# TheShadow29/VidSitu

Measured on AMD Instinct MI355X. Metric: clips/s (10s@32x224x224) SlowFast+TxEnc fwd+bwd, higher is better.
Workload: dtype bf16

## Files before the change

### vidsitu_amd/csrc/conv_stem.hip

```cpp
#include "common.h"

#define ST_TH 8
#define ST_TW 16
#define ST_PH 21
#define ST_PW 40
#define ST_ROWB (ST_PW * 8)
#define ST_FRAMEB (ST_PH * ST_ROWB)
#define ST_TC 4

struct StemP {
  const uint16_t* x;
  const uint16_t* w;
  uint16_t* y;
  const float* scale;
  const float* shift;
  float* stats;
  int N, T, H, W, Ho, Wo, Cout, kT, y_ld, flags;
  int tilesH, tilesW, tchunks, ntiles;
};

template <int NT>
__global__ __launch_bounds__(256) void stem_conv_kernel(StemP p) {
  extern __shared__ __attribute__((aligned(16))) char smem[];
  constexpr int CP = NT * 16;
  const int K = p.kT * 7 * 32;
  const int wpitch = K * 2 + 16;
  char* wlds = smem;
  char* patch = smem + ((CP * wpitch + 15) & ~15);
  const int patch_bytes = p.kT * ST_FRAMEB;
  float* E = (float*)(patch + ((patch_bytes + 15) & ~15));
  float* statbuf = E + 128 * CP;

  const int tid = threadIdx.x;
  {
    const int chunks_per_row = K / 8;
    for (int i = tid; i < CP * chunks_per_row; i += 256) {
      const int r = i / chunks_per_row, c = i - r * chunks_per_row;
      *(u32x4*)(wlds + r * wpitch + c * 16) = *(const u32x4*)(p.w + (long long)r * K + c * 8);
    }
  }
  const int wave = tid >> 6, lane = tid & 63;
  const int lr = lane & 15, lq = lane >> 4;
  const int pT = p.kT >> 1;

  auto stage_frame = [&](int n, int ti, int hi0, int wi0) __attribute__((always_inline)) {
    const int slot = ((ti % p.kT) + p.kT) % p.kT;
    char* dst = patch + slot * ST_FRAMEB;
    const bool tin = (unsigned)ti < (unsigned)p.T;
    const uint16_t* src = p.x + (((long long)n * p.T + (tin ? ti : 0)) * p.H) * (long long)p.W * 4;
    uint2 v[4];
#pragma unroll
    for (int u = 0; u < 4; ++u) {
      const int i = tid + u * 256;
      const int r = i / ST_PW, c = i - r * ST_PW;
      const int hi = hi0 + r, wi = wi0 + c;
      v[u] = make_uint2(0u, 0u);
      if (i < ST_PH * ST_PW && tin && (unsigned)hi < (unsigned)p.H && (unsigned)wi < (unsigned)p.W)
        v[u] = *(const uint2*)(src + ((long long)hi * p.W + wi) * 4);
    }
#pragma unroll
    for (int u = 0; u < 4; ++u) {
      const int i = tid + u * 256;
      if (i < ST_PH * ST_PW) *(uint2*)(dst + i * 8) = v[u];
    }
  };

  for (int item = blockIdx.x; item < p.ntiles; item += gridDim.x) {
    int t = item;
    const int tc = t % p.tchunks;
    t /= p.tchunks;
    const int tw = t % p.tilesW;
    t /= p.tilesW;
    const int th = t % p.tilesH;
    const int n = t / p.tilesH;
    const int ho0 = th * ST_TH, wo0 = tw * ST_TW;
    const int hi0 = 2 * ho0 - 3, wi0 = 2 * wo0 - 3;
    const int to_beg = tc * ST_TC, to_end = min(p.T, to_beg + ST_TC);
   for (int to = to_beg; to < to_end; ++to) {
    const int tile = ((n * p.T + to) * p.tilesH + th) * p.tilesW + tw;
    __syncthreads();
    if (to == to_beg) {
      for (int dt = 0; dt < p.kT; ++dt) stage_frame(n, to - pT + dt, hi0, wi0);
    } else {
      stage_frame(n, to + pT, hi0, wi0);
    }
    __syncthreads();

    f32x4 acc[2][NT];
#pragma unroll
    for (int a = 0; a < 2; ++a)
#pragma unroll
      for (int b = 0; b < NT; ++b) acc[a][b] = (f32x4){0.f, 0.f, 0.f, 0.f};

    int slot = (to - pT) % p.kT;
    if (slot < 0) slot += p.kT;
    int ks = 0;
    for (int dt = 0; dt < p.kT; ++dt) {
      const char* fbase = patch + slot * ST_FRAMEB + (2 * lr + 2 * lq) * 8;
      for (int dh = 0; dh < 7; ++dh, ++ks) {
        bf16x8 af[2], bfr[NT];
#pragma unroll
        for (int a = 0; a < 2; ++a) {
          const int hol = wave * 2 + a;
          af[a] = *(const bf16x8*)(fbase + (2 * hol + dh) * ST_ROWB);
        }
#pragma unroll
        for (int b = 0; b < NT; ++b)
          bfr[b] = *(const bf16x8*)(wlds + (b * 16 + lr) * wpitch + (ks * 32 + lq * 8) * 2);
#pragma unroll
        for (int a = 0; a < 2; ++a)
#pragma unroll
          for (int b = 0; b < NT; ++b)
            acc[a][b] = __builtin_amdgcn_mfma_f32_16x16x32_bf16(af[a], bfr[b], acc[a][b], 0, 0, 0);
      }
      if (++slot == p.kT) slot = 0;
    }

#pragma unroll
    for (int a = 0; a < 2; ++a) {
      const int ho = ho0 + wave * 2 + a;
#pragma unroll
      for (int r = 0; r < 4; ++r) {
        const int wo = wo0 + lq * 4 + r;
        if (ho >= p.Ho || wo >= p.Wo) {
#pragma unroll
          for (int b = 0; b < NT; ++b) acc[a][b][r] = 0.f;
        }
      }
    }
    if (p.flags & VS_CONV_STATS) {
#pragma unroll
      for (int b = 0; b < NT; ++b) {
        float s = 0.f, q = 0.f;
#pragma unroll
        for (int a = 0; a < 2; ++a)
#pragma unroll
          for (int r = 0; r < 4; ++r) {
            const float v = acc[a][b][r];
            s += v;
            q += v * v;
          }
        s += __shfl_xor(s, 16, 64);
        q += __shfl_xor(q, 16, 64);
        s += __shfl_xor(s, 32, 64);
        q += __shfl_xor(q, 32, 64);
        if (lq == 0) {
          statbuf[wave * CP + b * 16 + lr] = s;
          statbuf[4 * CP + wave * CP + b * 16 + lr] = q;
        }
      }
    }
#pragma unroll
    for (int b = 0; b < NT; ++b) {
      const int col = b * 16 + lr;
      float sc = 1.f, sh = 0.f;
      if ((p.flags & VS_CONV_AFFINE) && col < p.Cout) {
        sc = p.scale[col];
        sh = p.shift[col];
      }
#pragma unroll
      for (int a = 0; a < 2; ++a)
#pragma unroll
        for (int r = 0; r < 4; ++r) {
          const int row = (wave * 2 + a) * 16 + lq * 4 + r;
          E[row * CP + col] = acc[a][b][r] * sc + sh;
        }
    }
    __syncthreads();
    if ((p.flags & VS_CONV_STATS) && tid < p.Cout) {
      float s = 0.f, q = 0.f;
#pragma unroll
      for (int w = 0; w < 4; ++w) {
        s += statbuf[w * CP + tid];
        q += statbuf[4 * CP + w * CP + tid];
      }
      float* dst = p.stats + (long long)tile * 2 * p.Cout;
      dst[tid] = s;
      dst[p.Cout + tid] = q;
    }
    const int cpr = p.Cout >> 3;
    for (int idx = tid; idx < 128 * cpr; idx += 256) {
      const int row = idx / cpr, c8 = idx - row * cpr;
      const int ho = ho0 + (row >> 4), wo = wo0 + (row & 15);
      if (ho < p.Ho && wo < p.Wo) {
        float v[8];
        const float4 v0 = *(const float4*)(E + row * CP + c8 * 8);
        const float4 v1 = *(const float4*)(E + row * CP + c8 * 8 + 4);
        v[0] = v0.x; v[1] = v0.y; v[2] = v0.z; v[3] = v0.w;
        v[4] = v1.x; v[5] = v1.y; v[6] = v1.z; v[7] = v1.w;
        if (p.flags & VS_CONV_RELU) {
#pragma unroll
          for (int e = 0; e < 8; ++e) v[e] = fmaxf(v[e], 0.f);
        }
        const long long pos = (((long long)n * p.T + to) * p.Ho + ho) * p.Wo + wo;
        *(uint4*)(p.y + pos * p.y_ld + c8 * 8) = pack8_bf16(v);
      }
    }
   }
  }
}

#define SP_TH 16
#define SP_PH 37
#define SP_FRAMEB (SP_PH * ST_ROWB)
#define SP_TC 8

__global__ __launch_bounds__(512) void stem_pair_kernel(StemP p) {
  extern __shared__ __attribute__((aligned(16))) char smem[];
  const int kT = p.kT, KT1 = kT + 1, pT = kT >> 1;
  const int K = kT * 7 * 32, K2 = KT1 * 7 * 32;
  const int wpitch = K2 * 2 + 16;
  char* wlds = smem;
  char* patch = smem + ((16 * wpitch + 15) & ~15);
  float* E = (float*)(patch + ((KT1 * SP_FRAMEB + 15) & ~15));
  float* statbuf = E + 256 * 16;
  const int tid = threadIdx.x;
  {
    const int cpr = K2 / 8;
    for (int i = tid; i < 16 * cpr; i += 512) {
      const int r = i / cpr, c = i - r * cpr;
      const int ks = c >> 2, sub = c & 3;
      const int dtp = ks / 7, dh = ks - dtp * 7;
      const int j = r >> 3, co = r & 7, dt = dtp - j;
      u32x4 v = {0u, 0u, 0u, 0u};
      if (dt >= 0 && dt < kT && co < p.Cout)
        v = *(const u32x4*)(p.w + (long long)co * K + ((dt * 7 + dh) * 32 + sub * 8));
      *(u32x4*)(wlds + r * wpitch + c * 16) = v;
    }
  }
  const int wave = tid >> 6, lane = tid & 63;
  const int lr = lane & 15, lq = lane >> 4;
  const int tilesH16 = (p.Ho + SP_TH - 1) / SP_TH;

  auto slot_of = [&](int ti) { return ((ti % KT1) + KT1) % KT1; };
  auto frame_load = [&](int n, int ti, int hi0, int wi0, uint2* v) __attribute__((always_inline)) {
    const bool tin = (unsigned)ti < (unsigned)p.T;
    const uint16_t* src = p.x + (((long long)n * p.T + (tin ? ti : 0)) * p.H) * (long long)p.W * 4;
#pragma unroll
    for (int u = 0; u < 3; ++u) {
      const int i = tid + u * 512;
      const int r = i / ST_PW, c = i - r * ST_PW;
      const int hi = hi0 + r, wi = wi0 + c;
      v[u] = make_uint2(0u, 0u);
      if (i < SP_PH * ST_PW && tin && (unsigned)hi < (unsigned)p.H && (unsigned)wi < (unsigned)p.W)
        v[u] = *(const uint2*)(src + ((long long)hi * p.W + wi) * 4);
    }
  };
  auto frame_store = [&](int ti, const uint2* v) __attribute__((always_inline)) {
    char* dst = patch + slot_of(ti) * SP_FRAMEB;
#pragma unroll
    for (int u = 0; u < 3; ++u) {
      const int i = tid + u * 512;
      if (i < SP_PH * ST_PW) *(uint2*)(dst + i * 8) = v[u];
    }
  };

  for (int item = blockIdx.x; item < p.ntiles; item += gridDim.x) {
    int t = item;
    const int tc = t % p.tchunks;
    t /= p.tchunks;
    const int tw = t % p.tilesW;
    t /= p.tilesW;
    const int th = t % tilesH16;
    const int n = t / tilesH16;
    const int ho0 = th * SP_TH, wo0 = tw * ST_TW;
    const int hi0 = 2 * ho0 - 3, wi0 = 2 * wo0 - 3;
    const int to_beg = tc * SP_TC, to_end = min(p.T, to_beg + SP_TC);
    __syncthreads();
    for (int f = 0; f < KT1; ++f) {
      uint2 v[3];
      frame_load(n, to_beg - pT + f, hi0, wi0, v);
      frame_store(to_beg - pT + f, v);
    }
    __syncthreads();
    for (int to0 = to_beg; to0 < to_end; to0 += 2) {
      const bool more = to0 + 2 < to_end;
      uint2 nf0[3], nf1[3];
      if (more) {
        frame_load(n, to0 - pT + KT1, hi0, wi0, nf0);
        frame_load(n, to0 - pT + KT1 + 1, hi0, wi0, nf1);
      }
      f32x4 acc[2];
      acc[0] = (f32x4){0.f, 0.f, 0.f, 0.f};
      acc[1] = (f32x4){0.f, 0.f, 0.f, 0.f};
      int slot = slot_of(to0 - pT);
      const char* wrow = wlds + lr * wpitch + lq * 16;
      for (int dtp = 0; dtp < KT1; ++dtp) {
        const char* fbase = patch + slot * SP_FRAMEB + (2 * lr + 2 * lq) * 8 + (4 * wave) * ST_ROWB;
        bf16x8 af[9];
#pragma unroll
        for (int r = 0; r < 9; ++r) af[r] = *(const bf16x8*)(fbase + r * ST_ROWB);
#pragma unroll
        for (int dh = 0; dh < 7; ++dh) {
          const bf16x8 bfr = *(const bf16x8*)(wrow + (dtp * 7 + dh) * 64);
          acc[0] = __builtin_amdgcn_mfma_f32_16x16x32_bf16(af[dh], bfr, acc[0], 0, 0, 0);
          acc[1] = __builtin_amdgcn_mfma_f32_16x16x32_bf16(af[dh + 2], bfr, acc[1], 0, 0, 0);
        }
        if (++slot == KT1) slot = 0;
      }
      const int j = lr >> 3, co = lr & 7;
      const bool fok = to0 + j < p.T && co < p.Cout;
#pragma unroll
      for (int a = 0; a < 2; ++a) {
        const int ho = ho0 + wave * 2 + a;
#pragma unroll
        for (int r = 0; r < 4; ++r) {
          const int wo = wo0 + lq * 4 + r;
          if (ho >= p.Ho || wo >= p.Wo || !fok) acc[a][r] = 0.f;
        }
      }
      if (p.flags & VS_CONV_STATS) {
        float s = 0.f, q = 0.f;
#pragma unroll
        for (int a = 0; a < 2; ++a)
#pragma unroll
          for (int r = 0; r < 4; ++r) {
            const float v = acc[a][r];
            s += v;
            q += v * v;
          }
        s += __shfl_xor(s, 16, 64);
        q += __shfl_xor(q, 16, 64);
        s += __shfl_xor(s, 32, 64);
        q += __shfl_xor(q, 32, 64);
        if (lq == 0) {
          statbuf[wave * 16 + lr] = s;
          statbuf[8 * 16 + wave * 16 + lr] = q;
        }
      }
      {
        float sc = 1.f, sh = 0.f;
        if ((p.flags & VS_CONV_AFFINE) && co < p.Cout) {
          sc = p.scale[co];
          sh = p.shift[co];
        }
#pragma unroll
        for (int a = 0; a < 2; ++a)
#pragma unroll
          for (int r = 0; r < 4; ++r) E[((wave * 2 + a) * 16 + lq * 4 + r) * 16 + lr] = acc[a][r] * sc + sh;
      }
      __syncthreads();
      if ((p.flags & VS_CONV_STATS) && tid < 32) {
        const int h = tid >> 4, col = tid & 15, jj = col >> 3, cc = col & 7;
        const int th8 = 2 * th + h;
        if (cc < p.Cout && to0 + jj < p.T && th8 < p.tilesH) {
          float s = 0.f, q = 0.f;
#pragma unroll
          for (int w = 0; w < 4; ++w) {
            s += statbuf[(4 * h + w) * 16 + col];
            q += statbuf[8 * 16 + (4 * h + w) * 16 + col];
          }
          const int tile = ((n * p.T + to0 + jj) * p.tilesH + th8) * p.tilesW + tw;
          float* dst = p.stats + (long long)tile * 2 * p.Cout;
          dst[cc] = s;
          dst[p.Cout + cc] = q;
        }
      }
      {
        const int row = tid >> 1, jj = tid & 1;
        const int ho = ho0 + (row >> 4), wo = wo0 + (row & 15);
        if (ho < p.Ho && wo < p.Wo && to0 + jj < p.T) {
          float v[8];
          const float4 v0 = *(const float4*)(E + row * 16 + jj * 8);
          const float4 v1 = *(const float4*)(E + row * 16 + jj * 8 + 4);
          v[0] = v0.x; v[1] = v0.y; v[2] = v0.z; v[3] = v0.w;
          v[4] = v1.x; v[5] = v1.y; v[6] = v1.z; v[7] = v1.w;
          if (p.flags & VS_CONV_RELU) {
#pragma unroll
            for (int e = 0; e < 8; ++e) v[e] = fmaxf(v[e], 0.f);
          }
          const long long pos = (((long long)n * p.T + to0 + jj) * p.Ho + ho) * p.Wo + wo;
          *(uint4*)(p.y + pos * p.y_ld) = pack8_bf16(v);
        }
      }
      __syncthreads();
      if (more) {
        frame_store(to0 - pT + KT1, nf0);
        frame_store(to0 - pT + KT1 + 1, nf1);
      }
      __syncthreads();
    }
  }
}

template <int KT>
__global__ __launch_bounds__(256) void stem_pair_reg_kernel(StemP p) {
  extern __shared__ __attribute__((aligned(16))) char smem[];
  constexpr int KT1 = KT + 1, pT = KT >> 1, NKS = KT1 * 7;
  constexpr int K = KT * 7 * 32;
  char* patch = smem;
  float* E = (float*)(patch + ((KT1 * ST_FRAMEB + 15) & ~15));
  float* statbuf = E + 128 * 16;
  const int tid = threadIdx.x;
  const int wave = tid >> 6, lane = tid & 63;
  const int lr = lane & 15, lq = lane >> 4;
  const int j = lr >> 3, co = lr & 7;

  bf16x8 bfr[NKS];
#pragma unroll
  for (int ks = 0; ks < NKS; ++ks) {
    const int dtp = ks / 7, dh = ks - dtp * 7;
    const int dt = dtp - j;
    u32x4 v = {0u, 0u, 0u, 0u};
    if (dt >= 0 && dt < KT && co < p.Cout)
      v = *(const u32x4*)(p.w + (long long)co * K + ((dt * 7 + dh) * 32 + lq * 8));
    bfr[ks] = __builtin_bit_cast(bf16x8, v);
  }

  auto slot_of = [](int ti) { return ((ti % KT1) + KT1) % KT1; };
  auto frame_load = [&](int n, int ti, int hi0, int wi0, uint2* v) __attribute__((always_inline)) {
    const bool tin = (unsigned)ti < (unsigned)p.T;
    const uint16_t* src = p.x + (((long long)n * p.T + (tin ? ti : 0)) * p.H) * (long long)p.W * 4;
#pragma unroll
    for (int u = 0; u < 4; ++u) {
      const int i = tid + u * 256;
      const int r = i / ST_PW, c = i - r * ST_PW;
      const int hi = hi0 + r, wi = wi0 + c;
      v[u] = make_uint2(0u, 0u);
      if (i < ST_PH * ST_PW && tin && (unsigned)hi < (unsigned)p.H && (unsigned)wi < (unsigned)p.W)
        v[u] = *(const uint2*)(src + ((long long)hi * p.W + wi) * 4);
    }
  };
  auto frame_store = [&](int ti, const uint2* v) __attribute__((always_inline)) {
    char* dst = patch + slot_of(ti) * ST_FRAMEB;
#pragma unroll
    for (int u = 0; u < 4; ++u) {
      const int i = tid + u * 256;
      if (i < ST_PH * ST_PW) *(uint2*)(dst + i * 8) = v[u];
    }
  };

  for (int item = blockIdx.x; item < p.ntiles; item += gridDim.x) {
    int t = item;
    const int tc = t % p.tchunks;
    t /= p.tchunks;
    const int tw = t % p.tilesW;
    t /= p.tilesW;
    const int th = t % p.tilesH;
    const int n = t / p.tilesH;
    const int ho0 = th * ST_TH, wo0 = tw * ST_TW;
    const int hi0 = 2 * ho0 - 3, wi0 = 2 * wo0 - 3;
    const int to_beg = tc * SP_TC, to_end = min(p.T, to_beg + SP_TC);
    __syncthreads();
    for (int f = 0; f < KT1; ++f) {
      uint2 v[4];
      frame_load(n, to_beg - pT + f, hi0, wi0, v);
      frame_store(to_beg - pT + f, v);
    }
    __syncthreads();
    for (int to0 = to_beg; to0 < to_end; to0 += 2) {
      const bool more = to0 + 2 < to_end;
      uint2 nf0[4], nf1[4];
      if (more) {
        frame_load(n, to0 - pT + KT1, hi0, wi0, nf0);
        frame_load(n, to0 - pT + KT1 + 1, hi0, wi0, nf1);
      }
      f32x4 acc[2];
      acc[0] = (f32x4){0.f, 0.f, 0.f, 0.f};
      acc[1] = (f32x4){0.f, 0.f, 0.f, 0.f};
      int slot = slot_of(to0 - pT);
#pragma unroll
      for (int dtp = 0; dtp < KT1; ++dtp) {
        const char* fbase = patch + slot * ST_FRAMEB + (2 * lr + 2 * lq) * 8 + (4 * wave) * ST_ROWB;
        bf16x8 af[9];
#pragma unroll
        for (int r = 0; r < 9; ++r) af[r] = *(const bf16x8*)(fbase + r * ST_ROWB);
#pragma unroll
        for (int dh = 0; dh < 7; ++dh) {
          acc[0] = __builtin_amdgcn_mfma_f32_16x16x32_bf16(af[dh], bfr[dtp * 7 + dh], acc[0], 0, 0, 0);
          acc[1] = __builtin_amdgcn_mfma_f32_16x16x32_bf16(af[dh + 2], bfr[dtp * 7 + dh], acc[1], 0, 0, 0);
        }
        if (++slot == KT1) slot = 0;
      }
      const bool fok = to0 + j < p.T && co < p.Cout;
#pragma unroll
      for (int a = 0; a < 2; ++a) {
        const int ho = ho0 + wave * 2 + a;
#pragma unroll
        for (int r = 0; r < 4; ++r) {
          const int wo = wo0 + lq * 4 + r;
          if (ho >= p.Ho || wo >= p.Wo || !fok) acc[a][r] = 0.f;
        }
      }
      if (p.flags & VS_CONV_STATS) {
        float s = 0.f, q = 0.f;
#pragma unroll
        for (int a = 0; a < 2; ++a)
#pragma unroll
          for (int r = 0; r < 4; ++r) {
            const float v = acc[a][r];
            s += v;
            q += v * v;
          }
        s += __shfl_xor(s, 16, 64);
        q += __shfl_xor(q, 16, 64);
        s += __shfl_xor(s, 32, 64);
        q += __shfl_xor(q, 32, 64);
        if (lq == 0) {
          statbuf[wave * 16 + lr] = s;
          statbuf[4 * 16 + wave * 16 + lr] = q;
        }
      }
      {
        float sc = 1.f, sh = 0.f;
        if ((p.flags & VS_CONV_AFFINE) && co < p.Cout) {
          sc = p.scale[co];
          sh = p.shift[co];
        }
#pragma unroll
        for (int a = 0; a < 2; ++a)
#pragma unroll
          for (int r = 0; r < 4; ++r) E[((wave * 2 + a) * 16 + lq * 4 + r) * 16 + lr] = acc[a][r] * sc + sh;
      }
      __syncthreads();
      if ((p.flags & VS_CONV_STATS) && tid < 16) {
        const int jj = tid >> 3, cc = tid & 7;
        if (cc < p.Cout && to0 + jj < p.T) {
          float s = 0.f, q = 0.f;
#pragma unroll
          for (int w = 0; w < 4; ++w) {
            s += statbuf[w * 16 + tid];
            q += statbuf[4 * 16 + w * 16 + tid];
          }
          const int tile = ((n * p.T + to0 + jj) * p.tilesH + th) * p.tilesW + tw;
          float* dst = p.stats + (long long)tile * 2 * p.Cout;
          dst[cc] = s;
          dst[p.Cout + cc] = q;
        }
      }
      {
        const int row = tid >> 1, jj = tid & 1;
        const int ho = ho0 + (row >> 4), wo = wo0 + (row & 15);
        if (ho < p.Ho && wo < p.Wo && to0 + jj < p.T) {
          float v[8];
          const float4 v0 = *(const float4*)(E + row * 16 + jj * 8);
          const float4 v1 = *(const float4*)(E + row * 16 + jj * 8 + 4);
          v[0] = v0.x; v[1] = v0.y; v[2] = v0.z; v[3] = v0.w;
          v[4] = v1.x; v[5] = v1.y; v[6] = v1.z; v[7] = v1.w;
          if (p.flags & VS_CONV_RELU) {
#pragma unroll
            for (int e = 0; e < 8; ++e) v[e] = fmaxf(v[e], 0.f);
          }
          const long long pos = (((long long)n * p.T + to0 + jj) * p.Ho + ho) * p.Wo + wo;
          *(uint4*)(p.y + pos * p.y_ld) = pack8_bf16(v);
        }
      }
      __syncthreads();
      if (more) {
        frame_store(to0 - pT + KT1, nf0);
        frame_store(to0 - pT + KT1 + 1, nf1);
      }
      __syncthreads();
    }
  }
}

static size_t stem_pair_smem(int kT) {
  const int K2 = (kT + 1) * 7 * 32;
  const size_t w = ((size_t)16 * (K2 * 2 + 16) + 15) & ~(size_t)15;
  const size_t patch = ((size_t)(kT + 1) * SP_FRAMEB + 15) & ~(size_t)15;
  return w + patch + (size_t)256 * 16 * 4 + (size_t)2 * 8 * 16 * 4;
}

static size_t stem_smem(int CP, int kT) {
  const int K = kT * 7 * 32;
  const size_t w = ((size_t)CP * (K * 2 + 16) + 15) & ~(size_t)15;
  const size_t patch = ((size_t)kT * ST_FRAMEB + 15) & ~(size_t)15;
  return w + patch + (size_t)128 * CP * 4 + (size_t)2 * 4 * CP * 4;
}

extern "C" int vs_stem_stats_rows(int N, int T, int H, int W) {
  const int Ho = (H + 6 - 7) / 2 + 1, Wo = (W + 6 - 7) / 2 + 1;
  return N * T * ((Ho + ST_TH - 1) / ST_TH) * ((Wo + ST_TW - 1) / ST_TW);
}

extern "C" int vs_stem_conv_fwd(const void* x4, const void* wp, void* y, int N, int T, int H, int W,
                                int Cout, int kT, int y_ld, int flags, const float* scale,
                                const float* shift, float* stats_partial, void* stream) {
  VS_CHECK_ARG(x4 && wp && y, "null tensor");
  VS_CHECK_ARG(Cout % 8 == 0 && Cout <= 64 && y_ld % 8 == 0 && y_ld >= Cout, "Cout in {8..64}, pitch % 8");
  VS_CHECK_ARG(kT == 1 || kT == 3 || kT == 5, "kT in {1,3,5}");
  VS_CHECK_ARG(!(flags & VS_CONV_AFFINE) || (scale && shift), "AFFINE needs scale/shift");
  VS_CHECK_ARG(!(flags & VS_CONV_STATS) || stats_partial, "STATS needs stats_partial");
  VS_CHECK_ARG(!(flags & VS_CONV_RESIDUAL), "no residual on a stem");
  StemP p;
  p.x = (const uint16_t*)x4;
  p.w = (const uint16_t*)wp;
  p.y = (uint16_t*)y;
  p.scale = scale;
  p.shift = shift;
  p.stats = stats_partial;
  p.N = N; p.T = T; p.H = H; p.W = W;
  p.Ho = (H + 6 - 7) / 2 + 1;
  p.Wo = (W + 6 - 7) / 2 + 1;
  p.Cout = Cout; p.kT = kT; p.y_ld = y_ld; p.flags = flags;
  p.tilesH = (p.Ho + ST_TH - 1) / ST_TH;
  p.tilesW = (p.Wo + ST_TW - 1) / ST_TW;
  p.tchunks = (T + ST_TC - 1) / ST_TC;
  p.ntiles = N * p.tilesH * p.tilesW * p.tchunks;
  const int CP = (Cout + 15) / 16 * 16;
  hipStream_t st = (hipStream_t)stream;
  static const int pair_on = [] { const char* e = getenv("VS_STEM_PAIR"); return e ? atoi(e) : 1; }();
  if (pair_on == 1 && Cout == 8 && kT >= 3 && T >= 2) {
    p.tchunks = (T + SP_TC - 1) / SP_TC;
    p.ntiles = N * p.tilesH * p.tilesW * p.tchunks;
    const int grid2 = p.ntiles < 512 ? p.ntiles : 512;
    const size_t smem2 = (((size_t)(kT + 1) * ST_FRAMEB + 15) & ~(size_t)15) + (size_t)128 * 16 * 4 + 2 * 4 * 16 * 4;
    if (kT == 5) hipLaunchKernelGGL(stem_pair_reg_kernel<5>, dim3(grid2), dim3(256), smem2, st, p);
    else hipLaunchKernelGGL(stem_pair_reg_kernel<3>, dim3(grid2), dim3(256), smem2, st, p);
    VS_CHECK_LAUNCH();
    return VS_OK;
  }
  if (pair_on && Cout == 8 && kT >= 3 && T >= 2) {
    static bool attr_done = false;
    if (!attr_done) {
      (void)hipFuncSetAttribute((const void*)stem_pair_kernel, hipFuncAttributeMaxDynamicSharedMemorySize, 160 * 1024);
      attr_done = true;
    }
    p.tchunks = (T + SP_TC - 1) / SP_TC;
    p.ntiles = N * ((p.Ho + SP_TH - 1) / SP_TH) * p.tilesW * p.tchunks;
    const int grid2 = p.ntiles < 256 ? p.ntiles : 256;
    hipLaunchKernelGGL(stem_pair_kernel, dim3(grid2), dim3(512), stem_pair_smem(kT), st, p);
    VS_CHECK_LAUNCH();
    return VS_OK;
  }
  const size_t smem = stem_smem(CP, kT);
  int grid = p.ntiles < 512 ? p.ntiles : 512;
#define LAUNCH_STEM(NT_)                                                                         \
  do {                                                                                           \
    static bool attr_done = false;                                                               \
    if (!attr_done) {                                                                            \
      (void)hipFuncSetAttribute((const void*)stem_conv_kernel<NT_>,                              \
                                hipFuncAttributeMaxDynamicSharedMemorySize, 160 * 1024);         \
      attr_done = true;                                                                          \
    }                                                                                            \
    hipLaunchKernelGGL((stem_conv_kernel<NT_>), dim3(grid), dim3(256), smem, st, p);             \
  } while (0)
  switch (CP / 16) {
    case 1: LAUNCH_STEM(1); break;
    case 2: LAUNCH_STEM(2); break;
    case 3: LAUNCH_STEM(3); break;
    default: LAUNCH_STEM(4); break;
  }
#undef LAUNCH_STEM
  VS_CHECK_LAUNCH();
  return VS_OK;
}

typedef __attribute__((ext_vector_type(4))) short st_s16x4;
typedef __attribute__((address_space(3))) st_s16x4 st_lds_s16x4;
typedef __attribute__((ext_vector_type(8))) short st_s16x8;

__device__ __forceinline__ bf16x8 st_tr_pair(const char* p0, const char* p1) {
  const st_s16x4 lo = __builtin_amdgcn_ds_read_tr16_b64_v4i16((st_lds_s16x4*)p0);
  const st_s16x4 hi = __builtin_amdgcn_ds_read_tr16_b64_v4i16((st_lds_s16x4*)p1);
  const st_s16x8 v = __builtin_shufflevector(lo, hi, 0, 1, 2, 3, 4, 5, 6, 7);
  return __builtin_bit_cast(bf16x8, v);
}

struct StemWgP {
  const uint16_t* x;
  const uint16_t* dy;
  float* slabs;
  int N, T, H, W, Ho, Wo, Cout, kT, dy_ld;
  int tilesH, tilesW, tchunks, nitems;
};

template <int MT, int NTW>
__global__ __launch_bounds__(256) void stem_wgrad_kernel(StemWgP p) {
  extern __shared__ __attribute__((aligned(16))) char smem[];
  char* patch = smem;
  char* dyl = smem + ((p.kT * ST_FRAMEB + 15) & ~15);
  const int tid = threadIdx.x, wave = tid >> 6, lane = tid & 63;
  const int g = lane >> 4, li = lane & 15, q = li >> 2, p4 = li & 3;
  const int pT = p.kT >> 1;
  const int ntiles_n = p.kT * 14;

  f32x4 acc[MT][NTW];
  int nt_dt[NTW], nt_off[NTW];
#pragma unroll
  for (int b = 0; b < NTW; ++b) {
#pragma unroll
    for (int a = 0; a < MT; ++a) acc[a][b] = (f32x4){0.f, 0.f, 0.f, 0.f};
    const int nt = wave + 4 * b;
    const int half = nt & 1, row = nt >> 1;
    nt_dt[b] = row / 7;
    nt_off[b] = (row - nt_dt[b] * 7) * ST_ROWB + (half * 4 + p4) * 8;
  }

  auto stage_frame = [&](int n, int ti, int hi0, int wi0) __attribute__((always_inline)) {
    const int slot = ((ti % p.kT) + p.kT) % p.kT;
    char* dst = patch + slot * ST_FRAMEB;
    const bool tin = (unsigned)ti < (unsigned)p.T;
    const uint16_t* src = p.x + (((long long)n * p.T + (tin ? ti : 0)) * p.H) * (long long)p.W * 4;
    uint2 v[4];
#pragma unroll
    for (int u = 0; u < 4; ++u) {
      const int i = tid + u * 256;
      const int r = i / ST_PW, c = i - r * ST_PW;
      const int hi = hi0 + r, wi = wi0 + c;
      v[u] = make_uint2(0u, 0u);
      if (i < ST_PH * ST_PW && tin && (unsigned)hi < (unsigned)p.H && (unsigned)wi < (unsigned)p.W)
        v[u] = *(const uint2*)(src + ((long long)hi * p.W + wi) * 4);
    }
#pragma unroll
    for (int u = 0; u < 4; ++u) {
      const int i = tid + u * 256;
      if (i < ST_PH * ST_PW) *(uint2*)(dst + i * 8) = v[u];
    }
  };

  for (int item = blockIdx.x; item < p.nitems; item += gridDim.x) {
    int t = item;
    const int tc = t % p.tchunks;
    t /= p.tchunks;
    const int tw = t % p.tilesW;
    t /= p.tilesW;
    const int th = t % p.tilesH;
    const int n = t / p.tilesH;
    const int ho0 = th * ST_TH, wo0 = tw * ST_TW;
    const int hi0 = 2 * ho0 - 3, wi0 = 2 * wo0 - 3;
    const int to_beg = tc * ST_TC, to_end = min(p.T, to_beg + ST_TC);
    for (int to = to_beg; to < to_end; ++to) {
      __syncthreads();
      if (to == to_beg) {
        for (int dt = 0; dt < p.kT; ++dt) stage_frame(n, to - pT + dt, hi0, wi0);
      } else {
        stage_frame(n, to + pT, hi0, wi0);
      }
      for (int i = tid; i < MT * 128 * 2; i += 256) {
        const int h8 = i & 1;
        const int pos = (i >> 1) & 127;
        const int mt = i >> 8;
        const int ho = ho0 + (pos >> 4), wo = wo0 + (pos & 15);
        const int c = mt * 16 + h8 * 8;
        u32x4 v = {0u, 0u, 0u, 0u};
        if (ho < p.Ho && wo < p.Wo && c < p.Cout)
          v = *(const u32x4*)(p.dy + ((((long long)n * p.T + to) * p.Ho + ho) * p.Wo + wo) * p.dy_ld + c);
        *(u32x4*)(dyl + (mt * 128 + pos) * 32 + h8 * 16) = v;
      }
      __syncthreads();
      int slot0 = (to - pT) % p.kT;
      if (slot0 < 0) slot0 += p.kT;
#pragma unroll
      for (int ks = 0; ks < 4; ++ks) {
        const int k = ks * 32 + 8 * g + q;
        bf16x8 af[MT];
#pragma unroll
        for (int a = 0; a < MT; ++a) {
          const char* ptr = dyl + (a * 128 + k) * 32 + p4 * 8;
          af[a] = st_tr_pair(ptr, ptr + 4 * 32);
        }
        const int rowk = (2 * (k >> 4)) * ST_ROWB + (2 * (k & 15)) * 8;
#pragma unroll
        for (int b = 0; b < NTW; ++b) {
          if (wave + 4 * b < ntiles_n) {
            int sl = slot0 + nt_dt[b];
            if (sl >= p.kT) sl -= p.kT;
            const char* ptr = patch + sl * ST_FRAMEB + nt_off[b] + rowk;
            const bf16x8 bf = st_tr_pair(ptr, ptr + 4 * 16);
#pragma unroll
            for (int a = 0; a < MT; ++a)
              acc[a][b] = __builtin_amdgcn_mfma_f32_16x16x32_bf16(af[a], bf, acc[a][b], 0, 0, 0);
          }
        }
      }
    }
  }
  const int Kpad = p.kT * 7 * 32;
  float* dst = p.slabs + (long long)blockIdx.x * p.Cout * Kpad;
#pragma unroll
  for (int a = 0; a < MT; ++a)
#pragma unroll
    for (int b = 0; b < NTW; ++b) {
      const int nt = wave + 4 * b;
      if (nt < ntiles_n) {
#pragma unroll
        for (int r = 0; r < 4; ++r) {
          const int co = a * 16 + g * 4 + r;
          if (co < p.Cout) dst[(long long)co * Kpad + nt * 16 + li] = acc[a][b][r];
        }
      }
    }
}

template <int KT>
__global__ __launch_bounds__(256) void stem_wgrad_pair_kernel(StemWgP p) {
  extern __shared__ __attribute__((aligned(16))) char smem[];
  constexpr int KT1 = KT + 1, pT = KT >> 1;
  constexpr int NTN = KT1 * 14, NTW = (NTN + 3) / 4;
  char* patch = smem;
  char* dyl = smem + ((KT1 * ST_FRAMEB + 15) & ~15);
  const int tid = threadIdx.x, lane = tid & 63;
  const int wave = __builtin_amdgcn_readfirstlane(tid >> 6);
  const int g = lane >> 4, li = lane & 15, q = li >> 2, p4 = li & 3;

  f32x4 acc[NTW];
#pragma unroll
  for (int b = 0; b < NTW; ++b) acc[b] = (f32x4){0.f, 0.f, 0.f, 0.f};

  auto slot_of = [](int ti) { return ((ti % KT1) + KT1) % KT1; };
  auto frame_load = [&](int n, int ti, int hi0, int wi0, uint2* v) __attribute__((always_inline)) {
    const bool tin = (unsigned)ti < (unsigned)p.T;
    const uint16_t* src = p.x + (((long long)n * p.T + (tin ? ti : 0)) * p.H) * (long long)p.W * 4;
#pragma unroll
    for (int u = 0; u < 4; ++u) {
      const int i = tid + u * 256;
      const int r = i / ST_PW, c = i - r * ST_PW;
      const int hi = hi0 + r, wi = wi0 + c;
      v[u] = make_uint2(0u, 0u);
      if (i < ST_PH * ST_PW && tin && (unsigned)hi < (unsigned)p.H && (unsigned)wi < (unsigned)p.W)
        v[u] = *(const uint2*)(src + ((long long)hi * p.W + wi) * 4);
    }
  };
  auto frame_store = [&](int ti, const uint2* v) __attribute__((always_inline)) {
    char* dst = patch + slot_of(ti) * ST_FRAMEB;
#pragma unroll
    for (int u = 0; u < 4; ++u) {
      const int i = tid + u * 256;
      if (i < ST_PH * ST_PW) *(uint2*)(dst + i * 8) = v[u];
    }
  };
  auto dy_load = [&](int n, int to0, int ho0, int wo0) __attribute__((always_inline)) {
    const int jj = tid & 1, pos = tid >> 1;
    const int ho = ho0 + (pos >> 4), wo = wo0 + (pos & 15);
    u32x4 v = {0u, 0u, 0u, 0u};
    if (ho < p.Ho && wo < p.Wo && to0 + jj < p.T)
      v = *(const u32x4*)(p.dy + ((((long long)n * p.T + to0 + jj) * p.Ho + ho) * p.Wo + wo) * p.dy_ld);
    return v;
  };
  auto dy_store = [&](const u32x4& v) __attribute__((always_inline)) {
    *(u32x4*)(dyl + (tid >> 1) * 32 + (tid & 1) * 16) = v;
  };

  for (int item = blockIdx.x; item < p.nitems; item += gridDim.x) {
    int t = item;
    const int tc = t % p.tchunks;
    t /= p.tchunks;
    const int tw = t % p.tilesW;
    t /= p.tilesW;
    const int th = t % p.tilesH;
    const int n = t / p.tilesH;
    const int ho0 = th * ST_TH, wo0 = tw * ST_TW;
    const int hi0 = 2 * ho0 - 3, wi0 = 2 * wo0 - 3;
    const int to_beg = tc * SP_TC, to_end = min(p.T, to_beg + SP_TC);
    __syncthreads();
    for (int f = 0; f < KT1; ++f) {
      uint2 v[4];
      frame_load(n, to_beg - pT + f, hi0, wi0, v);
      frame_store(to_beg - pT + f, v);
    }
    dy_store(dy_load(n, to_beg, ho0, wo0));
    __syncthreads();
    for (int to0 = to_beg; to0 < to_end; to0 += 2) {
      const bool more = to0 + 2 < to_end;
      uint2 nf0[4], nf1[4];
      u32x4 ndy = {0u, 0u, 0u, 0u};
      if (more) {
        frame_load(n, to0 - pT + KT1, hi0, wi0, nf0);
        frame_load(n, to0 - pT + KT1 + 1, hi0, wi0, nf1);
        ndy = dy_load(n, to0 + 2, ho0, wo0);
      }
      const int slot0 = slot_of(to0 - pT);
#pragma unroll
      for (int ks = 0; ks < 4; ++ks) {
        const int k = ks * 32 + 8 * g + q;
        const char* aptr = dyl + k * 32 + p4 * 8;
        const bf16x8 af = st_tr_pair(aptr, aptr + 4 * 32);
        const char* bbase = patch + (2 * (k >> 4)) * ST_ROWB + (2 * (k & 15)) * 8 + p4 * 8;
#pragma unroll
        for (int b = 0; b < NTW; ++b) {
          const int nt = wave + 4 * b;
          if (nt < NTN) {
            const int half = nt & 1, row = nt >> 1;
            const int dtp = row / 7, dh = row - dtp * 7;
            int sl = slot0 + dtp;
            if (sl >= KT1) sl -= KT1;
            const char* ptr = bbase + sl * ST_FRAMEB + dh * ST_ROWB + half * 32;
            const bf16x8 bf = st_tr_pair(ptr, ptr + 4 * 16);
            acc[b] = __builtin_amdgcn_mfma_f32_16x16x32_bf16(af, bf, acc[b], 0, 0, 0);
          }
        }
      }
      __syncthreads();
      if (more) {
        frame_store(to0 - pT + KT1, nf0);
        frame_store(to0 - pT + KT1 + 1, nf1);
        dy_store(ndy);
      }
      __syncthreads();
    }
  }
  const int Kpad = KT * 7 * 32;
#pragma unroll
  for (int b = 0; b < NTW; ++b) {
    const int nt = wave + 4 * b;
    if (nt < NTN) {
#pragma unroll
      for (int r = 0; r < 4; ++r) {
        const int m = g * 4 + r, j = m >> 3, co = m & 7;
        const int ntd = nt - 14 * j;
        if (ntd >= 0 && ntd < KT * 14 && co < p.Cout) {
          float* dst = p.slabs + ((long long)blockIdx.x * 2 + j) * p.Cout * Kpad;
          dst[(long long)co * Kpad + ntd * 16 + li] = acc[b][r];
        }
      }
    }
  }
}

__global__ __launch_bounds__(256) void stem_slab_reduce_kernel(const float* slabs, float* dw,
                                                              long long n, int S) {
  __shared__ float4 part[16][17];
  const long long n4 = n >> 2;
  const int col = threadIdx.x & 15, sl = threadIdx.x >> 4;
  const long long i = (long long)blockIdx.x * 16 + col;
  float4 acc = make_float4(0.f, 0.f, 0.f, 0.f);
  if (i < n4) {
    const int per = (S + 15) / 16;
    const int s0 = sl * per, s1 = min(S, s0 + per);
    for (int s = s0; s < s1; ++s) {
      const float4 v = *(const float4*)(slabs + (long long)s * n + i * 4);
      acc.x += v.x; acc.y += v.y; acc.z += v.z; acc.w += v.w;
    }
  }
  part[sl][col] = acc;
  __syncthreads();
  if (sl == 0 && i < n4) {
    float4 t = part[0][col];
    for (int k = 1; k < 16; ++k) {
      const float4 v = part[k][col];
      t.x += v.x; t.y += v.y; t.z += v.z; t.w += v.w;
    }
    *(float4*)(dw + i * 4) = t;
  }
}

static int stem_wg_grid(int nitems) { return nitems < 512 ? nitems : 512; }

static bool stem_wg_pair(int T, int Cout, int kT) {
  static const int on = [] { const char* e = getenv("VS_STEM_PAIR"); return e ? atoi(e) : 1; }();
  return on && Cout == 8 && (kT == 3 || kT == 5) && T >= 2;
}

extern "C" size_t vs_stem_wgrad_workspace_bytes(int N, int T, int H, int W, int Cout, int kT) {
  const int Ho = (H + 6 - 7) / 2 + 1, Wo = (W + 6 - 7) / 2 + 1;
  const bool pair = stem_wg_pair(T, Cout, kT);
  const int tc = pair ? SP_TC : ST_TC;
  const int nitems = N * ((Ho + ST_TH - 1) / ST_TH) * ((Wo + ST_TW - 1) / ST_TW) * ((T + tc - 1) / tc);
  return (size_t)stem_wg_grid(nitems) * (pair ? 2 : 1) * Cout * kT * 7 * 32 * sizeof(float);
}

extern "C" int vs_stem_conv_wgrad(const void* dy, const void* x4, float* dwp, int N, int T, int H,
                                  int W, int Cout, int kT, int dy_ld, void* workspace,
                                  size_t ws_bytes, void* stream) {
  VS_CHECK_ARG(dy && x4 && dwp && workspace, "null tensor");
  VS_CHECK_ARG(Cout % 8 == 0 && Cout <= 64 && dy_ld % 8 == 0 && dy_ld >= Cout, "Cout in {8..64}, pitch % 8");
  VS_CHECK_ARG(kT == 1 || kT == 3 || kT == 5, "kT in {1,3,5}");
  StemWgP p;
  p.x = (const uint16_t*)x4;
  p.dy = (const uint16_t*)dy;
  p.slabs = (float*)workspace;
  p.N = N; p.T = T; p.H = H; p.W = W;
  p.Ho = (H + 6 - 7) / 2 + 1;
  p.Wo = (W + 6 - 7) / 2 + 1;
  p.Cout = Cout; p.kT = kT; p.dy_ld = dy_ld;
  p.tilesH = (p.Ho + ST_TH - 1) / ST_TH;
  p.tilesW = (p.Wo + ST_TW - 1) / ST_TW;
  p.tchunks = (T + ST_TC - 1) / ST_TC;
  p.nitems = N * p.tilesH * p.tilesW * p.tchunks;
  const int grid = stem_wg_grid(p.nitems);
  if (ws_bytes < vs_stem_wgrad_workspace_bytes(N, T, H, W, Cout, kT)) {
    vs_set_error("vs_stem_conv_wgrad: workspace too small");
    return VS_ERR_WORKSPACE;
  }
  const int MTv = (Cout + 15) / 16;
  hipStream_t st = (hipStream_t)stream;
  if (stem_wg_pair(T, Cout, kT)) {
    p.tchunks = (T + SP_TC - 1) / SP_TC;
    p.nitems = N * p.tilesH * p.tilesW * p.tchunks;
    const int grid2 = stem_wg_grid(p.nitems);
    const size_t smem2 = (((size_t)(kT + 1) * ST_FRAMEB + 15) & ~(size_t)15) + (size_t)128 * 32;
    if (kT == 5) hipLaunchKernelGGL(stem_wgrad_pair_kernel<5>, dim3(grid2), dim3(256), smem2, st, p);
    else hipLaunchKernelGGL(stem_wgrad_pair_kernel<3>, dim3(grid2), dim3(256), smem2, st, p);
    VS_CHECK_LAUNCH();
    const long long n2 = (long long)Cout * kT * 7 * 32;
    hipLaunchKernelGGL(stem_slab_reduce_kernel, dim3((unsigned)((n2 / 4 + 15) / 16)), dim3(256), 0, st,
                       (const float*)workspace, dwp, n2, 2 * grid2);
    VS_CHECK_LAUNCH();
    return VS_OK;
  }
  const size_t smem = (((size_t)kT * ST_FRAMEB + 15) & ~(size_t)15) + (size_t)MTv * 128 * 32;
  const int ntw = (kT * 14 + 3) / 4;
#define LAUNCH_SWG(MT_, NTW_)                                                                    \
  hipLaunchKernelGGL((stem_wgrad_kernel<MT_, NTW_>), dim3(grid), dim3(256), smem, st, p)
  if (MTv == 1 && ntw == 18) LAUNCH_SWG(1, 18);
  else if (MTv == 1 && ntw == 11) LAUNCH_SWG(1, 11);
  else if (MTv == 1) LAUNCH_SWG(1, 4);
  else if (MTv == 2 && ntw == 18) LAUNCH_SWG(2, 18);
  else if (MTv == 2 && ntw == 11) LAUNCH_SWG(2, 11);
  else if (MTv == 2) LAUNCH_SWG(2, 4);
  else if (MTv == 4 && ntw == 4) LAUNCH_SWG(4, 4);
  else if (MTv == 4 && ntw == 11) LAUNCH_SWG(4, 11);
  else if (MTv == 3 && ntw == 4) LAUNCH_SWG(3, 4);
  else {
    vs_set_error("vs_stem_conv_wgrad: unsupported (Cout, kT) = (%d, %d)", Cout, kT);
    return VS_ERR_UNSUPPORTED;
  }
#undef LAUNCH_SWG
  VS_CHECK_LAUNCH();
  const long long n = (long long)Cout * kT * 7 * 32;
  hipLaunchKernelGGL(stem_slab_reduce_kernel, dim3((unsigned)((n / 4 + 15) / 16)), dim3(256), 0, st,
                     (const float*)workspace, dwp, n, grid);
  VS_CHECK_LAUNCH();
  return VS_OK;
}
```

Baseline: 732.2.

## Replace stem wgrad pair kernel with async buffer-to-LDS ring pipeline

Rewrites the paired-frame stem weight-gradient kernel so that input patches and dy tiles are fetched with buffer_load ... lds DMA into a multi-stage LDS ring buffer. A persistent cursor walks items across the ring, and vmcnt waits plus a barrier replace the register-staged loads and double __syncthreads. This is meant to overlap global loads with the MFMA work and cut register pressure and sync overhead. The slab reduce kernel is also narrowed to 128 threads with an unrolled loop. The risks are tricky vmcnt accounting, out-of-bounds handling through an OOB offset sentinel, a 31-bit size limit, and higher LDS use.

```diff
diff --git a/vidsitu_amd/csrc/conv_stem.hip b/vidsitu_amd/csrc/conv_stem.hip
--- a/vidsitu_amd/csrc/conv_stem.hip
+++ b/vidsitu_amd/csrc/conv_stem.hip
@@ -664,6 +664,7 @@
   float* slabs;
   int N, T, H, W, Ho, Wo, Cout, kT, dy_ld;
   int tilesH, tilesW, tchunks, nitems;
+  unsigned x_bytes, dy_bytes;
 };
 
 template <int MT, int NTW>
@@ -784,114 +785,166 @@
     }
 }
 
-template <int KT>
-__global__ __launch_bounds__(256) void stem_wgrad_pair_kernel(StemWgP p) {
+#define SR_CPR 19
+#define SR_ROWB (SR_CPR * 16)
+#define SR_FCH (ST_PH * SR_CPR)
+#define SR_FRAMEB (SR_FCH * 16)
+#define SR_FP 13
+#define SR_STAGEB (SR_FP * 1024)
+#define SR_DYB 4096
+#define SR_NP (SR_FP + 4)
+#define SR_OOB 0x80000000u
+#define SR_DEPTH 2
+
+template <int N>
+__device__ __forceinline__ void sr_wait_vm() {
+  asm volatile("s_waitcnt vmcnt(%0)" ::"i"(N) : "memory");
+}
+
+struct SrCur {
+  int item;
+  int tp, tw, th, n;
+  int pro;
+  int left;
+};
+
+template <int KT, int D>
+__global__ __launch_bounds__(256) void stem_wgrad_ring_kernel(StemWgP p) {
   extern __shared__ __attribute__((aligned(16))) char smem[];
-  constexpr int KT1 = KT + 1, pT = KT >> 1;
-  constexpr int NTN = KT1 * 14, NTW = (NTN + 3) / 4;
-  char* patch = smem;
-  char* dyl = smem + ((KT1 * ST_FRAMEB + 15) & ~15);
+  constexpr int KT1 = KT + 1, pT = KT >> 1, NPRO = KT1 / 2 - 1, RS = NPRO + 1 + D, ND = D + 1;
+  constexpr int NTN = KT1 * 14, NTW = (NTN + 3) / 4, Kpad = KT * 7 * 32;
+  constexpr int LDSB = RS * SR_STAGEB + ND * SR_DYB;
+  static_assert((D - 1) * 5 <= 63, "vmcnt range");
   const int tid = threadIdx.x, lane = tid & 63;
-  const int wave = __builtin_amdgcn_readfirstlane(tid >> 6);
+  const int wave = __builtin_amdgcn_readfirstlane(tid >> 6) & 3;
   const int g = lane >> 4, li = lane & 15, q = li >> 2, p4 = li & 3;
+  const int TP = (p.T + 1) >> 1;
+  constexpr int PPI = SP_TC / 2;
+
+  for (int i = tid * 16; i < LDSB; i += 256 * 16) *(u32x4*)(smem + i) = (u32x4){0u, 0u, 0u, 0u};
+  __syncthreads();
 
   f32x4 acc[NTW];
 #pragma unroll
   for (int b = 0; b < NTW; ++b) acc[b] = (f32x4){0.f, 0.f, 0.f, 0.f};
 
-  auto slot_of = [](int ti) { return ((ti % KT1) + KT1) % KT1; };
-  auto frame_load = [&](int n, int ti, int hi0, int wi0, uint2* v) __attribute__((always_inline)) {
-    const bool tin = (unsigned)ti < (unsigned)p.T;
-    const uint16_t* src = p.x + (((long long)n * p.T + (tin ? ti : 0)) * p.H) * (long long)p.W * 4;
-#pragma unroll
-    for (int u = 0; u < 4; ++u) {
-      const int i = tid + u * 256;
-      const int r = i / ST_PW, c = i - r * ST_PW;
-      const int hi = hi0 + r, wi = wi0 + c;
-      v[u] = make_uint2(0u, 0u);
-      if (i < ST_PH * ST_PW && tin && (unsigned)hi < (unsigned)p.H && (unsigned)wi < (unsigned)p.W)
-        v[u] = *(const uint2*)(src + ((long long)hi * p.W + wi) * 4);
-    }
+  typedef __attribute__((address_space(3))) char* lds_ptr_t;
+  const unsigned lds0 = (unsigned)(unsigned long)(lds_ptr_t)smem;
+  auto rsrc_words = [](const void* base, unsigned bytes) __attribute__((always_inline)) {
+    const unsigned long a = (unsigned long)base;
+    return (i32x4){(int)(unsigned)a, (int)((unsigned)(a >> 32) & 0xffffu), (int)bytes, 0x00020000};
   };
-  auto frame_store = [&](int ti, const uint2* v) __attribute__((always_inline)) {
-    char* dst = patch + slot_of(ti) * ST_FRAMEB;
-#pragma unroll
-    for (int u = 0; u < 4; ++u) {
-      const int i = tid + u * 256;
-      if (i < ST_PH * ST_PW) *(uint2*)(dst + i * 8) = v[u];
-    }
+  const i32x4 xdesc = rsrc_words(p.x, p.x_bytes), dydesc = rsrc_words(p.dy, p.dy_bytes);
+  auto dma16 = [](const i32x4& desc, unsigned lds_addr, unsigned voff) __attribute__((always_inline)) {
+    asm volatile("s_mov_b32 m0, %0\n\ts_nop 0\n\tbuffer_load_dwordx4 %1, %2, 0 offen lds"
+                 :
+                 : "s"(lds_addr), "v"(voff), "s"(desc)
+                 : "memory");
   };
-  auto dy_load = [&](int n, int to0, int ho0, int wo0) __attribute__((always_inline)) {
-    const int jj = tid & 1, pos = tid >> 1;
-    const int ho = ho0 + (pos >> 4), wo = wo0 + (pos & 15);
-    u32x4 v = {0u, 0u, 0u, 0u};
-    if (ho < p.Ho && wo < p.Wo && to0 + jj < p.T)
-      v = *(const u32x4*)(p.dy + ((((long long)n * p.T + to0 + jj) * p.Ho + ho) * p.Wo + wo) * p.dy_ld);
-    return v;
-  };
-  auto dy_store = [&](const u32x4& v) __attribute__((always_inline)) {
-    *(u32x4*)(dyl + (tid >> 1) * 32 + (tid & 1) * 16) = v;
-  };
-
-  for (int item = blockIdx.x; item < p.nitems; item += gridDim.x) {
+
+  auto seek = [&](SrCur& c, int item) __attribute__((always_inline)) {
+    c.item = item;
     int t = item;
     const int tc = t % p.tchunks;
     t /= p.tchunks;
-    const int tw = t % p.tilesW;
+    c.tw = t % p.tilesW;
     t /= p.tilesW;
-    const int th = t % p.tilesH;
-    const int n = t / p.tilesH;
-    const int ho0 = th * ST_TH, wo0 = tw * ST_TW;
-    const int hi0 = 2 * ho0 - 3, wi0 = 2 * wo0 - 3;
-    const int to_beg = tc * SP_TC, to_end = min(p.T, to_beg + SP_TC);
-    __syncthreads();
-    for (int f = 0; f < KT1; ++f) {
-      uint2 v[4];
-      frame_load(n, to_beg - pT + f, hi0, wi0, v);
-      frame_store(to_beg - pT + f, v);
-    }
-    dy_store(dy_load(n, to_beg, ho0, wo0));
-    __syncthreads();
-    for (int to0 = to_beg; to0 < to_end; to0 += 2) {
-      const bool more = to0 + 2 < to_end;
-      uint2 nf0[4], nf1[4];
-      u32x4 ndy = {0u, 0u, 0u, 0u};
-      if (more) {
-        frame_load(n, to0 - pT + KT1, hi0, wi0, nf0);
-        frame_load(n, to0 - pT + KT1 + 1, hi0, wi0, nf1);
-        ndy = dy_load(n, to0 + 2, ho0, wo0);
-      }
-      const int slot0 = slot_of(to0 - pT);
+    c.th = t % p.tilesH;
+    c.n = t / p.tilesH;
+    c.tp = tc * PPI;
+    c.left = min(PPI, TP - c.tp);
+    c.pro = NPRO;
+  };
+  auto advance = [&](SrCur& c) __attribute__((always_inline)) {
+    if (c.pro > 0) {
+      --c.pro;
+      return;
+    }
+    ++c.tp;
+    if (--c.left == 0) seek(c, c.item + (int)gridDim.x);
+  };
+  auto issue = [&](const SrCur& c, int reg, int dys) __attribute__((always_inline)) {
+    const bool valid = c.item < p.nitems;
+    const int to0 = 2 * c.tp;
+    const int f0 = to0 - pT + 2 * (NPRO - c.pro);
+    const int hi0 = 2 * (c.th * ST_TH) - 3, wi0 = 2 * (c.tw * ST_TW) - 4;
+    const int ho0 = c.th * ST_TH, wo0 = c.tw * ST_TW;
+#pragma unroll
+    for (int u = 0; u < (SR_NP + 3) / 4; ++u) {
+      const int i = wave + 4 * u;
+      if (i < SR_FP) {
+        const int ch = i * 64 + lane;
+        const int f = ch >= SR_FCH ? 1 : 0, cc = ch - f * SR_FCH;
+        const int r = cc / SR_CPR, col = cc - r * SR_CPR;
+        const int ti = f0 + f, hi = hi0 + r, wi = wi0 + 2 * col;
+        const bool ok = valid & (ch < 2 * SR_FCH) & ((unsigned)ti < (unsigned)p.T) & ((unsigned)hi < (unsigned)p.H) &
+                        ((unsigned)wi < (unsigned)p.W);
+        const unsigned off = ok ? ((unsigned)(((c.n * p.T + ti) * p.H + hi) * p.W + wi) << 3) : SR_OOB;
+        dma16(xdesc, lds0 + (unsigned)(reg * SR_STAGEB + i * 1024), off);
+      } else if (i < SR_NP) {
+        const int ch = (i - SR_FP) * 64 + lane;
+        const int jj = ch & 1, pos = ch >> 1;
+        const int ho = ho0 + (pos >> 4), wo = wo0 + (pos & 15);
+        const bool ok = valid & (c.pro == 0) & (ho < p.Ho) & (wo < p.Wo) & (to0 + jj < p.T);
+        const unsigned off =
+            ok ? (unsigned)(((c.n * p.T + to0 + jj) * p.Ho + ho) * p.Wo + wo) * (unsigned)(p.dy_ld * 2) : SR_OOB;
+        dma16(dydesc, lds0 + (unsigned)(RS * SR_STAGEB + dys * SR_DYB + (i - SR_FP) * 1024), off);
+      }
+    }
+  };
+
+  SrCur cc;
+  seek(cc, blockIdx.x);
+  SrCur ld = cc;
+  int l_reg = 0, l_dy = 0, c_reg = 0, c_dy = 0;
+#pragma unroll
+  for (int d = 0; d < D; ++d) {
+    issue(ld, l_reg, l_dy);
+    advance(ld);
+    l_reg = l_reg + 1 == RS ? 0 : l_reg + 1;
+    l_dy = l_dy + 1 == ND ? 0 : l_dy + 1;
+  }
+  while (cc.item < p.nitems) {
+    if (wave == 0) sr_wait_vm<(D - 1) * 5>();
+    else sr_wait_vm<(D - 1) * 4>();
+    __builtin_amdgcn_s_barrier();
+    __builtin_amdgcn_sched_barrier(0);
+    issue(ld, l_reg, l_dy);
+    advance(ld);
+    l_reg = l_reg + 1 == RS ? 0 : l_reg + 1;
+    l_dy = l_dy + 1 == ND ? 0 : l_dy + 1;
+    __builtin_amdgcn_sched_barrier(0);
+    if (cc.pro == 0) {
+      int r0 = c_reg - NPRO;
+      if (r0 < 0) r0 += RS;
+      const char* dyl = smem + RS * SR_STAGEB + c_dy * SR_DYB;
 #pragma unroll
       for (int ks = 0; ks < 4; ++ks) {
         const int k = ks * 32 + 8 * g + q;
         const char* aptr = dyl + k * 32 + p4 * 8;
         const bf16x8 af = st_tr_pair(aptr, aptr + 4 * 32);
-        const char* bbase = patch + (2 * (k >> 4)) * ST_ROWB + (2 * (k & 15)) * 8 + p4 * 8;
+        const char* bbase = smem + (2 * (k >> 4)) * SR_ROWB + (2 * (k & 15) + 1) * 8 + p4 * 8;
 #pragma unroll
         for (int b = 0; b < NTW; ++b) {
           const int nt = wave + 4 * b;
           if (nt < NTN) {
             const int half = nt & 1, row = nt >> 1;
             const int dtp = row / 7, dh = row - dtp * 7;
-            int sl = slot0 + dtp;
-            if (sl >= KT1) sl -= KT1;
-            const char* ptr = bbase + sl * ST_FRAMEB + dh * ST_ROWB + half * 32;
+            int rg = r0 + (dtp >> 1);
+            if (rg >= RS) rg -= RS;
+            const char* ptr = bbase + rg * SR_STAGEB + (dtp & 1) * SR_FRAMEB + dh * SR_ROWB + half * 32;
             const bf16x8 bf = st_tr_pair(ptr, ptr + 4 * 16);
             acc[b] = __builtin_amdgcn_mfma_f32_16x16x32_bf16(af, bf, acc[b], 0, 0, 0);
           }
         }
       }
-      __syncthreads();
-      if (more) {
-        frame_store(to0 - pT + KT1, nf0);
-        frame_store(to0 - pT + KT1 + 1, nf1);
-        dy_store(ndy);
-      }
-      __syncthreads();
-    }
-  }
-  const int Kpad = KT * 7 * 32;
+    }
+    __builtin_amdgcn_sched_barrier(0);
+    advance(cc);
+    c_reg = c_reg + 1 == RS ? 0 : c_reg + 1;
+    c_dy = c_dy + 1 == ND ? 0 : c_dy + 1;
+  }
+  sr_wait_vm<0>();
 #pragma unroll
   for (int b = 0; b < NTW; ++b) {
     const int nt = wave + 4 * b;
@@ -909,16 +962,17 @@
   }
 }
 
-__global__ __launch_bounds__(256) void stem_slab_reduce_kernel(const float* slabs, float* dw,
+__global__ __launch_bounds__(128) void stem_slab_reduce_kernel(const float* slabs, float* dw,
                                                               long long n, int S) {
-  __shared__ float4 part[16][17];
+  __shared__ float4 part[16][9];
   const long long n4 = n >> 2;
-  const int col = threadIdx.x & 15, sl = threadIdx.x >> 4;
-  const long long i = (long long)blockIdx.x * 16 + col;
+  const int col = threadIdx.x & 7, sl = threadIdx.x >> 3;
+  const long long i = (long long)blockIdx.x * 8 + col;
   float4 acc = make_float4(0.f, 0.f, 0.f, 0.f);
   if (i < n4) {
     const int per = (S + 15) / 16;
     const int s0 = sl * per, s1 = min(S, s0 + per);
+#pragma unroll 8
     for (int s = s0; s < s1; ++s) {
       const float4 v = *(const float4*)(slabs + (long long)s * n + i * 4);
       acc.x += v.x; acc.y += v.y; acc.z += v.z; acc.w += v.w;
@@ -938,17 +992,23 @@
 
 static int stem_wg_grid(int nitems) { return nitems < 512 ? nitems : 512; }
 
-static bool stem_wg_pair(int T, int Cout, int kT) {
+static bool stem_wg_ring(int N, int T, int H, int W, int Cout, int kT, int dy_ld) {
   static const int on = [] { const char* e = getenv("VS_STEM_PAIR"); return e ? atoi(e) : 1; }();
-  return on && Cout == 8 && (kT == 3 || kT == 5) && T >= 2;
+  const long long Ho = (H + 6 - 7) / 2 + 1, Wo = (W + 6 - 7) / 2 + 1;
+  const long long xb = (long long)N * T * H * W * 8, dyb = (long long)N * T * Ho * Wo * dy_ld * 2;
+  return on && Cout == 8 && (kT == 3 || kT == 5) && T >= 2 && W % 2 == 0 && xb < (1ll << 31) && dyb < (1ll << 31);
 }
 
 extern "C" size_t vs_stem_wgrad_workspace_bytes(int N, int T, int H, int W, int Cout, int kT) {
   const int Ho = (H + 6 - 7) / 2 + 1, Wo = (W + 6 - 7) / 2 + 1;
-  const bool pair = stem_wg_pair(T, Cout, kT);
-  const int tc = pair ? SP_TC : ST_TC;
-  const int nitems = N * ((Ho + ST_TH - 1) / ST_TH) * ((Wo + ST_TW - 1) / ST_TW) * ((T + tc - 1) / tc);
-  return (size_t)stem_wg_grid(nitems) * (pair ? 2 : 1) * Cout * kT * 7 * 32 * sizeof(float);
+  const long long tiles = (long long)N * ((Ho + ST_TH - 1) / ST_TH) * ((Wo + ST_TW - 1) / ST_TW);
+  const long long a = tiles * ((T + ST_TC - 1) / ST_TC), b = tiles * ((T + SP_TC - 1) / SP_TC);
+  size_t slabs = (size_t)stem_wg_grid((int)(a < 512 ? a : 512));
+  if (stem_wg_ring(N, T, H, W, Cout, kT, Cout)) {
+    const size_t s2 = 2 * (size_t)stem_wg_grid((int)(b < 512 ? b : 512));
+    slabs = s2 > slabs ? s2 : slabs;
+  }
+  return slabs * Cout * kT * 7 * 32 * sizeof(float);
 }
 
 extern "C" int vs_stem_conv_wgrad(const void* dy, const void* x4, float* dwp, int N, int T, int H,
@@ -969,6 +1029,7 @@
   p.tilesW = (p.Wo + ST_TW - 1) / ST_TW;
   p.tchunks = (T + ST_TC - 1) / ST_TC;
   p.nitems = N * p.tilesH * p.tilesW * p.tchunks;
+  p.x_bytes = p.dy_bytes = 0;
   const int grid = stem_wg_grid(p.nitems);
   if (ws_bytes < vs_stem_wgrad_workspace_bytes(N, T, H, W, Cout, kT)) {
     vs_set_error("vs_stem_conv_wgrad: workspace too small");
@@ -976,16 +1037,30 @@
   }
   const int MTv = (Cout + 15) / 16;
   hipStream_t st = (hipStream_t)stream;
-  if (stem_wg_pair(T, Cout, kT)) {
+  if (stem_wg_ring(N, T, H, W, Cout, kT, dy_ld)) {
     p.tchunks = (T + SP_TC - 1) / SP_TC;
     p.nitems = N * p.tilesH * p.tilesW * p.tchunks;
+    p.x_bytes = (unsigned)((long long)N * T * H * W * 8);
+    p.dy_bytes = (unsigned)((long long)N * T * p.Ho * p.Wo * dy_ld * 2);
     const int grid2 = stem_wg_grid(p.nitems);
-    const size_t smem2 = (((size_t)(kT + 1) * ST_FRAMEB + 15) & ~(size_t)15) + (size_t)128 * 32;
-    if (kT == 5) hipLaunchKernelGGL(stem_wgrad_pair_kernel<5>, dim3(grid2), dim3(256), smem2, st, p);
-    else hipLaunchKernelGGL(stem_wgrad_pair_kernel<3>, dim3(grid2), dim3(256), smem2, st, p);
+    constexpr int D = SR_DEPTH;
+    const size_t smem2 = (size_t)((kT + 1) / 2 + D) * SR_STAGEB + (size_t)(D + 1) * SR_DYB;
+#define LAUNCH_RING(KT_)                                                                         \
+  do {                                                                                           \
+    static bool attr_done = false;                                                               \
+    if (!attr_done) {                                                                            \
+      (void)hipFuncSetAttribute((const void*)stem_wgrad_ring_kernel<KT_, D>,                     \
+                                hipFuncAttributeMaxDynamicSharedMemorySize, 160 * 1024);         \
+      attr_done = true;                                                                          \
+    }                                                                                            \
+    hipLaunchKernelGGL((stem_wgrad_ring_kernel<KT_, D>), dim3(grid2), dim3(256), smem2, st, p);  \
+  } while (0)
+    if (kT == 5) LAUNCH_RING(5);
+    else LAUNCH_RING(3);
+#undef LAUNCH_RING
     VS_CHECK_LAUNCH();
     const long long n2 = (long long)Cout * kT * 7 * 32;
-    hipLaunchKernelGGL(stem_slab_reduce_kernel, dim3((unsigned)((n2 / 4 + 15) / 16)), dim3(256), 0, st,
+    hipLaunchKernelGGL(stem_slab_reduce_kernel, dim3((unsigned)((n2 / 4 + 7) / 8)), dim3(128), 0, st,
                        (const float*)workspace, dwp, n2, 2 * grid2);
     VS_CHECK_LAUNCH();
     return VS_OK;
@@ -1010,7 +1085,7 @@
 #undef LAUNCH_SWG
   VS_CHECK_LAUNCH();
   const long long n = (long long)Cout * kT * 7 * 32;
-  hipLaunchKernelGGL(stem_slab_reduce_kernel, dim3((unsigned)((n / 4 + 15) / 16)), dim3(256), 0, st,
+  hipLaunchKernelGGL(stem_slab_reduce_kernel, dim3((unsigned)((n / 4 + 7) / 8)), dim3(128), 0, st,
                      (const float*)workspace, dwp, n, grid);
   VS_CHECK_LAUNCH();
   return VS_OK;
```

Result: no change. 739.4, median of 6 (+1.0%).
